# FrancisTheCat/raytracing_c

Measured on AMD Instinct MI355X. Metric: Mray/s, higher is better.
Workload: dtype f32; 1 GPU; helmet.glb 1920x1080, 256 spp, 8 bounces (BASELINE.json configs[2]); partition=single GPU

## Files before the change

### include/rt_hip.h

```cpp
#ifndef RT_HIP_H
#define RT_HIP_H

#include "rt_raytracer.h"
#include "rt_materials.h"

#ifdef __cplusplus
extern "C" {
#endif

extern char const *rt_last_error(void);
extern void        rt_clear_error(void);

extern int rt_init(int device);

extern int rt_set_devices(i32 n_devices, i32 rehearse);
extern i32 rt_device_count(void);


extern void rt_set_seed(u32 seed);
extern u32  rt_get_seed(void);


typedef struct RT_Device_Scene RT_Device_Scene;

// ... 207 lines not shown

extern i64 rt_guided_upsample_work_bytes(i32 width, i32 height);
extern int rt_guided_upsample(i32 width, i32 height, RT_Upsample_Params const *params, void const *d_color_low,
                              void const *d_coverage_low, void const *d_albedo_low, void const *d_normal_low,
                              void const *d_position_low, void const *d_coverage, void const *d_albedo, void const *d_normal,
                              void const *d_position, void *d_out, void *d_image, void *d_work, void *stream);
extern int rt_guided_upsample_host(i32 width, i32 height, RT_Upsample_Params const *params, f32 const *color_low,
                                   RT_Features const *low, RT_Features const *full, f32 *out, u8 *image);
extern int rt_render_upsampled(Scene const *scene, Image const *image, isize samples, isize max_bounces,
                               RT_Upsample_Params const *upsample_params, RT_Guided_Params const *guided_params, f32 *linear_low,
                               f32 *linear_upsampled, f32 *linear_out);


extern int rt_render_accumulate_chunks(RT_Device_Scene *dscene, RT_Render_Params const *params, i32 n_list, i32 const *chunks,
                                       void *d_accum, void *stream);
extern int rt_adaptive_merge(i32 width, i32 height, i32 n, i32 n_list, i32 const *chunks, void *d_accum, void *d_fresh, void *d_err,
                             void *stream);
extern int rt_resolve_adaptive(i32 width, i32 height, void const *d_chunk_samples, void const *d_accum, void *d_image, void *d_linear,
                               void *d_sample_map, void *stream);

typedef struct {
  i32 min_samples;
  i32 max_samples;
  f32 threshold;
  i32 reserved;
} RT_Adaptive_Params;

extern int rt_render_adaptive(Scene const *scene, Image const *image, RT_Adaptive_Params const *ap, isize max_bounces, f32 *linear,
                              u64 *accum, i32 *chunk_samples);

extern int rt_get_counters(RT_Counters *out);
extern int rt_get_skipped_root_visits(u64 *out);
extern int rt_get_leafless_paths(u64 *out);
extern int rt_get_fused_root_visits(u64 *out);
extern int rt_get_shade_taps_form(void);
extern int rt_materials_share_taps(f32 const *mats, i32 n_materials);

typedef struct {
  f32 stamp_ms, upload_ms, enqueue_ms, gpu_prep_ms, gpu_path_ms, gpu_resolve_ms, gpu_copy_ms, total_ms;
  f32 verify_ms;
  f32 gather_ms;
  i32 n_devices;
  i32 slowest_device;
} RT_Frame_Timing;
extern int rt_get_frame_timing(RT_Frame_Timing *out);

extern f32 rt_last_kernel_ms(void);

extern void rt_kernel_timing_reset(void);
extern f32  rt_kernel_timing_mean_ms(i32 *n_launches);

extern int rt_math_contract(void);


#ifdef __cplusplus
}
#endif

#endif
```

### raytracing_c_amd/csrc/rt_dev.hip.h

```cpp
#ifndef RT_DEV_HIP_H
#define RT_DEV_HIP_H

#include <hip/hip_runtime.h>
#include <stdint.h>

#include "rt_device.h"
#include "../../include/rt_math.h"

#define RT_BLOCK_WAVES 4
#define RT_BLOCK_THREADS (RT_BLOCK_WAVES * 64)

struct Ray3 {
  rt_v3 o, d;
  float inv_x, inv_y, inv_z;
  bool  fast;
};

__device__ __forceinline__ rt_v3 slab_bias3(const Ray3 &r) {
#ifdef RT_MATH_NO_FMA
  return rt_v3_make(0.0f, 0.0f, 0.0f);
#else
  float px, py, pz;
  asm volatile("v_mul_f32 %0, %1, %2" : "=v"(px) : "v"(r.o.x), "v"(r.inv_x));
  asm volatile("v_mul_f32 %0, %1, %2" : "=v"(py) : "v"(r.o.y), "v"(r.inv_y));
// ... 1201 lines not shown
  surv &= surv - 1u;
  const int k2 = (int)__builtin_ctz(surv);
  const int e2 = as_i(slab_entry_ordered(r, bs, nbase, k2, nx, ny, nz, hit_t));
  const uint32_t f2 = 1u - (((uint32_t)e2 + 0x00800000u) >> 31);
  int e3 = 0x7F800000, k3 = 0;
  uint32_t f3 = 0;
  LGM_FEW("four_begin");
  if (n == 4) {
    surv &= surv - 1u;
    k3 = (int)__builtin_ctz(surv);
      e3 = as_i(slab_entry_ordered(r, bs, nbase, k3, nx, ny, nz, hit_t));
    f3 = 1u - (((uint32_t)e3 + 0x00800000u) >> 31);
  }
  LGM_FEW("four_end");
  const int e[4] = {e0, e1, e2, e3};
  const int kk[4] = {k0, k1, k2, k3};
  int rank[4] = {0, 1, 2, 3};
#pragma unroll
  for (int j = 0; j < 4; j++) {
#pragma unroll
    for (int k = j + 1; k < 4; k++) {
      int kb = (int)((uint32_t)(e[k] - e[j]) >> 31);
      rank[j] += kb;
      rank[k] -= kb;
    }
  }
  uint32_t w = 0;
#pragma unroll
  for (int j = 0; j < 4; j++) w |= (uint32_t)kk[j] << (3 * rank[j]);
  return w | ((f0 + f1 + f2 + f3) << 24);
}
#undef LGM_FEW

__device__ __forceinline__ uint32_t pyramid_cull_tris(const float *leaves, const float *pyr, int g) {
  const int lane = lane_now();
  const float *tb = leaves + (size_t)g * 72 + (lane & 7);
  const float *pl = pyr + RT_PYR_PLANE + ((lane >> 3) & 3) * 4;
  const float ox = pyr[RT_PYR_ORIGIN], oy = pyr[RT_PYR_ORIGIN + 1], oz = pyr[RT_PYR_ORIGIN + 2];
  const float nx = pl[0], ny = pl[1], nz = pl[2];
  const float ax = tb[0], e1x = tb[8], e2x = tb[16], ay = tb[24], e1y = tb[32], e2y = tb[40], az = tb[48], e1z = tb[56], e2z = tb[64];
  const float band = 2.5f * RT_EPS * (fabsf(nx * e1x + ny * e1y + nz * e1z) + fabsf(nx * e2x + ny * e2y + nz * e2z));
  bool outside = true;
#pragma unroll
  for (int v = 0; v < 3; v++) {
    const float vx = v == 0 ? ax : (v == 1 ? ax + e1x : ax + e2x);
    const float vy = v == 0 ? ay : (v == 1 ? ay + e1y : ay + e2y);
    const float vz = v == 0 ? az : (v == 1 ? az + e1z : az + e2z);
    const float px = nx * (vx - ox), py = ny * (vy - oy), pz = nz * (vz - oz);
    const float val = px + py + pz;
    const float extent = fabsf(px) + fabsf(py) + fabsf(pz);
    const float coarse = fabsf(nx) * (fabsf(ox) + fabsf(vx)) + fabsf(ny) * (fabsf(oy) + fabsf(vy)) + fabsf(nz) * (fabsf(oz) + fabsf(vz));
    outside = outside && (val - band > 1e-3f * extent + 1e-6f * coarse);
  }
  const uint32_t m = (uint32_t)__ballot(outside);
  return (m | (m >> 8) | (m >> 16) | (m >> 24)) & 0xFFu;
}

template <bool SHORT_DIV>
__device__ __forceinline__ void tri_test_uniform(const Ray3 &r, rt_v3 a, rt_v3 edge1, rt_v3 edge2, int k, float &best, float &bu, float &bv, int &bi) {
  rt_v3 rxe2 = rt_v3_cross(r.d, edge2);
  float det = rt_v3_dot(edge1, rxe2);
  float inv_det = SHORT_DIV ? rcp_leaf(det) : 1.0f / det;
  rt_v3 s = rt_v3_sub(r.o, a);
  rt_v3 sxe1 = rt_v3_cross(s, edge1);
  float u = inv_det * rt_v3_dot(s, rxe2);
  float v = inv_det * rt_v3_dot(r.d, sxe1);
  float t = inv_det * rt_v3_dot(edge2, sxe1);
  bool miss = (u < -RT_EPS) || (u > 1.0f + RT_EPS) || (v < -RT_EPS) || (u + v > 1.0f + RT_EPS) || (t < RT_EPS);
  if (SHORT_DIV) {
    if (!miss && t < best) { best = t; bi = k; bu = u; bv = v; }
  } else {
    float dist = miss ? RT_INF : t;
    dist = (dist > 0.0f) ? dist : RT_INF;
    if (dist < best) { best = dist; bi = k; bu = u; bv = v; }
  }
}
template <bool SHORT_DIV>
__device__ __forceinline__ bool leaf_test_uniform(const RT_KParams &P, const Ray3 &r, int g, uint32_t surv, HitRec &hit) {
  float best = RT_INF, bu = 0.0f, bv = 0.0f;
  int   bi = 0;
  cfloat *lb = as_scalar_ptr(P.leaves) + (size_t)g * 72;
  while (surv) {
    const int k0 = (int)__builtin_ctz(surv);
    surv &= surv - 1u;
    cfloat *t0 = lb + k0;
    tri_test_uniform<SHORT_DIV>(r, rt_v3_make(t0[0], t0[24], t0[48]), rt_v3_make(t0[8], t0[32], t0[56]), rt_v3_make(t0[16], t0[40], t0[64]),
                                k0, best, bu, bv, bi);
// ... 336 lines not shown
```

### raytracing_c_amd/csrc/rt_device.h

```cpp
#ifndef RT_DEVICE_H
#define RT_DEVICE_H

#include <stdint.h>

#define RT_NODE_F4   12
#define RT_LEAF_F4   18
#define RT_TRI_F4     7
#define RT_MAT_F4     9
#define RT_MAT_FLOATS 36
#define RT_MAX_DEPTH  8

#define RT_LDS_BYTES            (160 * 1024)
#define RT_LDS_NODE_BYTES       208
#define RT_LDS_TABLE_BYTES      64
#define RT_LDS_PERM_LEVEL_BYTES 256
#define RT_LDS_ACC_TILE_BYTES   1536

#define RT_MAT_DISNEY 0
#define RT_MAT_DEBUG  1

#define RT_TILE      8
#define RT_TILE_PIX  64

#define RT_PARK_RECORD_DWORDS (18 * 128)
enum {
  RT_CNT_PATHS = 0, RT_CNT_RAYS, RT_CNT_NODES, RT_CNT_LEAVES, RT_CNT_SHADES, RT_CNT_BG, RT_CNT_TEXTURED,
  RT_CNT_SKIPPED_ROOT,
  RT_CNT_LEDGER,
  RT_CNT_LEAFLESS = 136,
  RT_CNT_FUSED_ROOT,
  RT_N_COUNTERS
};
#define RT_CNT_LEDGER_SLOTS (RT_CNT_LEAFLESS - RT_CNT_LEDGER)



typedef struct {
  uint32_t offset;
  int32_t  width, height, stride;
} RT_DTexture;
#define RT_TEX_TILE_INDEX(x, y, tpr) ((((y) >> 2) * (tpr) + ((x) >> 2)) * 16 + (((y) & 3) << 2) + ((x) & 3))

typedef struct RT_KView {
  float    cam[3][4];
  float    focal_length;
  uint32_t seed;
  uint32_t pad[2];
} RT_KView;

typedef struct {
  const float    *nodes;
  const float    *leaves;
  const float    *tris;
  const float    *mats;
  const RT_DTexture *textures;
  const uint32_t *texels;
  int32_t depth;
  int32_t last_row_offset;
  int32_t bg_texture;
  int32_t n_nodes;
  float cam[3][4];
  float focal_length;
  float inv_width, inv_height, aspect;
// ... 101 lines not shown
```

### raytracing_c_amd/csrc/rt_kernels.hip

```cpp

#include "rt_dev.hip.h"


#ifdef RT_LEDGER
#define RT_LEDGER_WAVES 8192
__device__ uint32_t g_ledger[RT_LEDGER_WAVES * RT_LEDGER_ROW];
__global__ void rt_ledger_reduce_kernel(unsigned long long *counters) {
  const int slot = threadIdx.x;
  if (slot >= LG_N || slot >= RT_LEDGER_ROW) return;
  unsigned long long sum = 0ull;
  for (int w = 0; w < RT_LEDGER_WAVES; w++) sum += g_ledger[w * RT_LEDGER_ROW + slot];
  counters[RT_CNT_LEDGER + slot] = sum;
}
#endif

template <int WAVES, bool LDSN, int MIN_WAVES_PER_SIMD, bool SHORT_DIV, bool VIEWS, bool SHARED_TAPS>
__global__ __launch_bounds__(WAVES * 64, MIN_WAVES_PER_SIMD) void rt_path_kernel_stream(RT_KParams P) {
  extern __shared__ float4 smem[];
  const int lane = threadIdx.x & 63;
  const int wave = threadIdx.x >> 6;
  const int n_lds = LDSN ? P.n_lds_nodes : 0;
  const float4 *lds_nodes = smem;
  const WaveLds L = wave_lds(smem, n_lds, P.depth, wave);
  unsigned long long *acc = L.acc;
// ... 43 lines not shown
  const int leaf_level = P.depth - 1;
  const int thresh = P.sched_thresh;
  const int drain_thresh = P.drain_thresh;
  const int pyr_nodes = LDSN ? P.pyr_nodes : 0;
  const int wave_id = (int)blockIdx.x * WAVES + wave;

  bool queue_open = true;
  int  steal_tries = 0;

  for (;;) {
    LGT0();
    LGM("tile_begin");
    int tile_idx = queue_open ? take_queue_tile(lane, queue_open) : -1;
    if (tile_idx < 0) {
      if (steal_tries >= RT_STEAL_TRIES) break;
      steal_tries += 1;
      LG(LG_JOIN_X, 1);
      tile_idx = join_open_tile(lane, wave_id, steal_tries, n_chunks_tile LG_ARG);
      if (tile_idx < 0) break;
    }

    int tile_x0, tile_y0;
    RT_KViewP vrec = nullptr;
    if (!tile_origin<VIEWS>(lane, tile_idx, n_chunks_tile, tile_x0, tile_y0, vrec)) continue;
    bool tile_root_miss = false;
    if (leaf_level >= 0) {
      typename CamSrc<VIEWS>::type S;
      if constexpr (VIEWS) S = vrec; else S = cold_args();
      tile_root_miss = tile_pyramid(S, P.nodes, smem, pyr_off, lane, tile_x0, tile_y0);
    }
    int n_list = 0;
    int ll_levels = leaf_level, ll_nodes = pyr_nodes, ll_leaf0 = P.last_row_offset;
    asm volatile("" : "+s"(ll_levels), "+s"(ll_nodes), "+s"(ll_leaf0));
    if (ll_levels >= 1 && ll_nodes > 0 && !tile_root_miss) n_list = leafless_walk(smem, lds_nodes, pyr_off, ll_levels, ll_nodes, ll_leaf0);
    const uint32_t rays_before = w_rays;
    LG(LG_TILE_X, 1);
    LGM("tile_end");
    LGT1(LG_CYC_TILE);

    int   pix = 0, bounce = 0;
    uint32_t rng = 0;
    Ray3  ray;
    ray_setup(ray, rt_v3_make(0, 0, 0), rt_v3_make(0, 0, 1));
    rt_v3 tint = rt_v3_make(1, 1, 1), emis = rt_v3_make(0, 0, 0);
    TravState T = RT_TRAV_IDLE;

    bool tile_open = true;
    TileUnits U;
    tile_units_init(U, queue_open);
    int  n_parked = 0;
    uint32_t *park = cold_args()->park;

    if ((tile_root_miss || n_list > 0) && cold_args()->max_bounces > 0) {
      RT_KArgs A = cold_args();
      typename CamSrc<VIEWS>::type S;
      if constexpr (VIEWS) S = vrec; else S = A;
      const int width = A->width, height = A->height, sample_first = A->sample_first, sample_end = A->sample_end;
      const uint32_t n_sb = (uint32_t)A->n_sample_blocks, gmax = (uint32_t)A->grab_max;
      PrimaryParams PP;
      primary_params(PP, S, A);
      ShadeParamsLds SP;
      shade_params(SP, A, false);
      uint32_t *tile_next = A->tile_next, *open_groups = A->open_groups;
      uint32_t n_sky = 0;
      const uint32_t *list = leafless_list(smem, pyr_off, ll_levels);
      const uint32_t list_entry = (n_list > 1 && lane_now() < n_list) ? list[RT_LL_ENTRY + (lane_now() & (RT_LL_MAX - 1))] : 0u;
      for (;;) {
        if (U.c_next >= U.c_end) {
          if (U.u_cur + 1u < U.u_end) {
            U.u_cur += 1u;
          } else {
            uint32_t u0 = 0;
            if (lane == 0) u0 = atomicAdd(&tile_next[tile_idx], U.grab);
            u0 = (uint32_t)__builtin_amdgcn_readfirstlane((int)u0);
            if (u0 >= n_chunks_tile) { tile_open = false; break; }
            U.u_cur = u0;
            U.u_end = u0 + U.grab < n_chunks_tile ? u0 + U.grab : n_chunks_tile;
            if (U.u_end == n_chunks_tile && lane == 0) atomicSub(&open_groups[tile_idx >> 6], 1u);
            if (t_wave_start) t_last_grab = __builtin_amdgcn_s_memrealtime();
            LG(LG_GRAB_X, 1);
            const uint32_t left = n_chunks_tile - U.u_end;
            U.grab = left >= 8u * gmax ? gmax : (left >= 8u && gmax >= 2u ? 2u : 1u);
            U.took_any = true;
          }
          unit_decode(U, tile_x0, tile_y0, shift, unit_paths, n_sb, sample_first, width, height);
          continue;
        }
#ifndef RT_SKY_PATHS
#define RT_SKY_PATHS 1
#endif
        LGM("sky_begin");
        LGT0();
        const int avail = U.c_end - U.c_next;
        const int take = avail < 64 * RT_SKY_PATHS ? avail : 64 * RT_SKY_PATHS;
        const int l = lane_now();
        bool valid[RT_SKY_PATHS];
        int  pxs[RT_SKY_PATHS];
        rt_v3 dirs[RT_SKY_PATHS];
        Ray3 rs[RT_SKY_PATHS];
        bool slow = false;
#pragma unroll
        for (int q = 0; q < RT_SKY_PATHS; q++) {
          const int kq = l + 64 * q;
          const int k = U.c_next + kq;
          pxs[q] = k >> shift;
          const int sm = U.c_s0 + (k & ((1 << shift) - 1));
          const int x = U.c_x0 + pxs[q];
          valid[q] = kq < take && x < width && sm < sample_end;
          rt_v3 o = rt_v3_make(0, 0, 0);
          dirs[q] = rt_v3_make(0, 0, 1);
          if (valid[q]) primary_ray(PP, x, U.c_y, sm, o, dirs[q]);
          ray_setup<SHORT_DIV>(rs[q], o, dirs[q]);
          slow = slow || (valid[q] && !rs[q].fast);
        }
        if (__ballot(slow) != 0ull) break;
        uint32_t nv = 0;
        uint32_t e = (uint32_t)__builtin_amdgcn_readlane((int)list_entry, 1);
        if ((int)e < 0) {
#pragma unroll
          for (int q = 0; q < RT_SKY_PATHS; q++) {
            const Ray3 &r = rs[q];
            const int nx = (as_i(r.inv_x) >> 31) & 96, ny = (as_i(r.inv_y) >> 31) & 96, nz = (as_i(r.inv_z) >> 31) & 96;
            const rt_v3 bs = slab_bias3(r);
            uint32_t entered = valid[q] ? 1u : 0u;
            int i = 1;
            if (q > 0) e = (uint32_t)__builtin_amdgcn_readlane((int)list_entry, 1);
            do {
              const char *cb = reinterpret_cast<const char *>(lds_nodes) + (e & 0xFFFFFu);
              const float t = slab_entry_ordered(r, bs, cb, 0, nx, ny, nz, RT_INF);
              const uint32_t in = ((entered >> ((e >> 20) & 7u)) & 1u) & (t < RT_INF ? 1u : 0u);
              entered |= in << i;
              w_nodes += (uint32_t)__popcll(__ballot(in != 0u));
              i += 1;
              e = (uint32_t)__builtin_amdgcn_readlane((int)list_entry, i);
            } while ((int)e < 0);
          }
        }
#pragma unroll
        for (int q = 0; q < RT_SKY_PATHS; q++) {
          unsigned long long qr = 0ull, qg = 0ull, qb = 0ull;
          if (valid[q]) {
            const rt_v3 bg = background_lookup(SP, dirs[q]);
            const rt_v3 radiance = rt_v3_mul_add(bg, rt_v3_make(1, 1, 1), rt_v3_make(0, 0, 0));
            qr = accum_quantize_dev(radiance.x); qg = accum_quantize_dev(radiance.y); qb = accum_quantize_dev(radiance.z);
          }
          tile_add_samples_grouped(smem, acc_off, U.c_pix0 + pxs[q], U.c_end >= 2 * RT_SKY_ADD_GROUP, valid[q], qr, qg, qb);
          nv += (uint32_t)__popcll(__ballot(valid[q]));
        }
        w_paths += nv; w_rays += nv; w_nodes += nv; w_bgs += nv;
        n_sky += nv;
        LG(LG_SKY_X, 1); LG(LG_SKY_L, nv);
        U.c_next += take;
        LGT1(LG_CYC_SKY);
        LGM("sky_end");
      }
      if (n_sky != 0u && lane == 0) atomicAdd(cold_args()->counters + (tile_root_miss ? RT_CNT_SKIPPED_ROOT : RT_CNT_LEAFLESS), (unsigned long long)n_sky);
    }

    for (;;) {
      {
        LGT0();
        LGM("s_begin");
        LG(LG_S_ITER, 1);
        LaneCounters cn;
        cn.rays = cn.nodes = cn.leaves = cn.shades = cn.bgs = cn.textured = cn.paths = 0;
        bool  done = false, start = false, fresh = false;
        rt_v3 radiance = rt_v3_make(0, 0, 0);
        rt_v3 org = ray.o, dir = ray.d;
        RT_KArgs A = cold_args();
        typename PathShadeParams<SHARED_TAPS>::type SP;
        shade_params(SP, A, true);
#ifdef RT_LEDGER
        { const int n_env = (int)__popcll(__ballot(T.phase == PH_MISS)); LG(LG_ENV_X, n_env != 0); LG(LG_ENV_L, n_env); }
#endif
        LGM("env_begin");
        if (T.phase == PH_MISS) {
          cn.bgs = 1;
          rt_v3 bg = background_lookup(SP, dir);
          radiance = rt_v3_mul_add(bg, tint, emis);
          done = true;
        }
        LGM("env_end");
        bool shade_now = true;
        if (park) {
          const unsigned long long mHit = __ballot(T.phase == PH_HIT);
          const unsigned long long mIdle = __ballot(T.phase == PH_NEED) | __ballot(T.phase == PH_MISS);
          const int h = (int)__popcll(mHit), f = (int)__popcll(mIdle);
          const int back = n_parked < f ? n_parked : f;
          uint32_t *pk = park + (size_t)__builtin_amdgcn_readfirstlane(wave_id) * (RT_PARK_FIELDS * RT_PARK_CAP);
// ... 669 lines not shown
```

### raytracing_c_amd/csrc/rt_launch.cpp

```cpp

#include "rt_host.h"

static std::atomic<int> g_taps_form{-1};

int check_params(RT_Render_Params const *p) {
  if (!p) return rt_fail("render params are NULL");
  if (p->width <= 0 || p->height <= 0) return rt_fail("image size %dx%d is invalid", p->width, p->height);
  if ((int64_t)p->width * p->height > (int64_t)1 << 28) return rt_fail("image %dx%d is too large", p->width, p->height);
  if (p->samples <= 0) return rt_fail("samples must be positive (got %d)", p->samples);
  if (p->max_bounces < 0) return rt_fail("max_bounces must be >= 0 (got %d)", p->max_bounces);
  if (p->world <= 0 || p->rank < 0 || p->rank >= p->world) return rt_fail("rank %d / world %d is invalid", p->rank, p->world);
  if (p->sample_first < 0 || p->sample_count < 0 || p->sample_first + p->sample_count > p->samples)
    return rt_fail("sample range [%d, +%d) outside [0, %d)", p->sample_first, p->sample_count, p->samples);
  return 0;
}

int check_image_size(const char *who, i32 width, i32 height) {
  if (width <= 0 || height <= 0) return rt_fail("%s: image size %dx%d is invalid", who, width, height);
  if ((int64_t)width * height > RT_MAX_PIXELS) return rt_fail("%s: image %dx%d is too large (more than 2^28 pixels)", who, width, height);
  return 0;
}

int check_views(i32 n_views, RT_View const *views, i32 width, i32 height, const char *who) {
  if (n_views <= 0) return rt_fail("%s: n_views must be positive (got %d)", who, n_views);
// ... 418 lines not shown

int copy_image_out(Image const *image, const uint8_t *d_image, int width, int height, hipStream_t stream) {
  size_t pixels = (size_t)width * height;
  if (!image->pixels.data) return 0;
  if (image->components == 3 && image->stride == image->width) {
    HIP_TRY(hipMemcpyAsync(image->pixels.data, d_image, pixels * 3, hipMemcpyDeviceToHost, stream));
    HIP_TRY(hipStreamSynchronize(stream));
  } else {
    std::vector<uint8_t> tmp(pixels * 3);
    HIP_TRY(hipMemcpy(tmp.data(), d_image, pixels * 3, hipMemcpyDeviceToHost));
    for (isize y = 0; y < image->height; y++)
      for (isize x = 0; x < image->width; x++)
        for (int c = 0; c < 3; c++)
          image->pixels.data[image->components * (x + y * image->stride) + c] = tmp[((size_t)y * width + x) * 3 + c];
  }
  return 0;
}

static int get_counter(const char *who, int index, u64 *out) {
  if (!out) return rt_fail("%s: NULL", who);
  Device &D = dev0();
  std::lock_guard<std::mutex> lock(D.mutex);
  if (ensure_device(D) != 0) return -1;
  unsigned long long c[RT_N_COUNTERS];
  if (read_counters(D, c) != 0) return -1;
  *out = c[index];
  return 0;
}

extern "C" int rt_get_skipped_root_visits(u64 *out) { return get_counter("rt_get_skipped_root_visits", RT_CNT_SKIPPED_ROOT, out); }

extern "C" int rt_get_leafless_paths(u64 *out) { return get_counter("rt_get_leafless_paths", RT_CNT_LEAFLESS, out); }

extern "C" int rt_get_fused_root_visits(u64 *out) { return get_counter("rt_get_fused_root_visits", RT_CNT_FUSED_ROOT, out); }

extern "C" int rt_get_shade_taps_form(void) { return g_taps_form.load(); }

int read_counters(Device &D, unsigned long long c[RT_N_COUNTERS]) {
  HIP_TRY(hipDeviceSynchronize());
  if (!D.last_counters) { memset(c, 0, RT_N_COUNTERS * sizeof(unsigned long long)); return 0; }
  HIP_TRY(hipMemcpy(c, D.last_counters, RT_N_COUNTERS * sizeof(unsigned long long), hipMemcpyDeviceToHost));
  return 0;
}

extern "C" int rt_get_counters(RT_Counters *out) {
  if (!out) return rt_fail("rt_get_counters: NULL");
  {
    std::lock_guard<std::mutex> lk(g_multi_mutex);
    if (g_multi_counters_valid) { *out = g_multi_counters; return 0; }
  }
  Device &D = dev0();
  std::lock_guard<std::mutex> lock(D.mutex);
  if (ensure_device(D) != 0) return -1;
  unsigned long long c[RT_N_COUNTERS];
  if (read_counters(D, c) != 0) return -1;
  out->paths = c[RT_CNT_PATHS];
  out->rays = c[RT_CNT_RAYS];
  out->node_visits = c[RT_CNT_NODES];
  out->leaf_visits = c[RT_CNT_LEAVES];
  out->shades = c[RT_CNT_SHADES];
  out->backgrounds = c[RT_CNT_BG];
  out->textured = c[RT_CNT_TEXTURED];
  return 0;
}

static float timed_slot_ms(Workspace &W, size_t slot) {
// ... 34 lines not shown
```

### raytracing_c_amd/csrc/rt_tile.hip.h

```cpp
#ifndef RT_TILE_HIP_H
#define RT_TILE_HIP_H

typedef const RT_KView __attribute__((address_space(4))) *RT_KViewP;
template <bool VIEWS> struct CamSrc { typedef RT_KArgs type; };
template <> struct CamSrc<true> { typedef RT_KViewP type; };

__device__ __forceinline__ int take_queue_tile(const int lane, bool &queue_open) {
  RT_KArgs A = cold_args();
  uint32_t pos = 0;
  if (lane == 0) pos = atomicAdd(A->work_head, 1u);
  pos = (uint32_t)__builtin_amdgcn_readfirstlane((int)pos);
  const uint32_t *order = A->order;
  if (pos < (uint32_t)A->n_tiles) return order ? (int)order[pos] : (int)pos;
  queue_open = false;
  return -1;
}

__device__ __forceinline__ int join_open_tile(const int lane, const int wave_id, const int steal_tries, const uint32_t n_chunks_tile,
                                              uint32_t *lg = nullptr) {
  LGT0();
  int tile_idx = -1;
  RT_KArgs A = cold_args();
  const int n_tiles = A->n_tiles;
  const uint32_t *open_groups = A->open_groups, *tile_next = A->tile_next;
// ... 91 lines not shown
  for (int q = 0; q < 4; q++) {
    rt_v3 n = rt_v3_cross(c[q], c[(q + 1) & 3]);
    if (rt_v3_dot(n, c[(q + 2) & 3]) > 0.0f) n = rt_v3_scale(n, -1.0f);
    pn[q] = n;
  }
  float *pyr = lds_at(smem, pyr_off);
  if (lane == 0) {
#pragma unroll
    for (int q = 0; q < 4; q++) { pyr[RT_PYR_PLANE + q * 4 + 0] = pn[q].x; pyr[RT_PYR_PLANE + q * 4 + 1] = pn[q].y; pyr[RT_PYR_PLANE + q * 4 + 2] = pn[q].z; }
    pyr[RT_PYR_ORIGIN] = o.x; pyr[RT_PYR_ORIGIN + 1] = o.y; pyr[RT_PYR_ORIGIN + 2] = o.z;
  }
  if (lane < RT_PYR_CACHE_WORDS) reinterpret_cast<uint32_t *>(pyr)[RT_PYR_LEAF_CACHE + lane] = 0u;
  bool may_hit = false;
  if (lane < 8) {
    const float *nb = nodes + lane;
    rt_v3 lo = rt_v3_make(nb[0] - o.x, nb[8] - o.y, nb[16] - o.z);
    rt_v3 hi = rt_v3_make(nb[24] - o.x, nb[32] - o.y, nb[40] - o.z);
    bool outside = child_box_empty(nb);
#pragma unroll
    for (int q = 0; q < 4; q++) {
      rt_v3 n = pn[q];
      float lox = n.x * lo.x, hix = n.x * hi.x, loy = n.y * lo.y, hiy = n.y * hi.y, loz = n.z * lo.z, hiz = n.z * hi.z;
      float nearest = fminf(lox, hix) + fminf(loy, hiy) + fminf(loz, hiz);
      float extent = fmaxf(fabsf(lox), fabsf(hix)) + fmaxf(fabsf(loy), fabsf(hiy)) + fmaxf(fabsf(loz), fabsf(hiz));
      float coarse = fabsf(n.x) * (fabsf(o.x) + fmaxf(fabsf(nb[0]), fabsf(nb[24]))) + fabsf(n.y) * (fabsf(o.y) + fmaxf(fabsf(nb[8]), fabsf(nb[32]))) +
                     fabsf(n.z) * (fabsf(o.z) + fmaxf(fabsf(nb[16]), fabsf(nb[40])));
      if (nearest > 1e-3f * extent + 1e-6f * coarse) outside = true;
    }
    may_hit = !outside;
  }
  return __ballot(may_hit) == 0ull;
}

#define RT_LL_MAX   8
#define RT_LL_ENTRY 0
#define RT_LL_NODE  RT_LL_MAX
__device__ __forceinline__ uint32_t *leafless_list(float4 *smem, const int pyr_off, const int levels) {
  return reinterpret_cast<uint32_t *>(lds_at(smem, pyr_off) - levels * (RT_LDS_PERM_LEVEL_BYTES / 4));
}
__device__ __forceinline__ int leafless_walk(float4 *smem, const float4 *lds_nodes, const int pyr_off, const int levels, const int n_nodes,
                                             const int leaf0) {
  const float *pyr = lds_at(smem, pyr_off);
  uint32_t *list = leafless_list(smem, pyr_off, levels);
  int n_list = 1;
  for (int head = 0; head < n_list; head++) {
    const int nd = head ? __builtin_amdgcn_readfirstlane((int)list[RT_LL_NODE + head]) : 0;
    const uint32_t surv = 0xFFu & ~pyramid_cull_mask(lds_nodes, pyr, nd);
    if (lane_now() == 0) reinterpret_cast<uint32_t *>(lds_at(smem, pyr_off))[RT_PYR_NODE_CACHE + (nd & 31)] = ((uint32_t)(nd + 1) << 8) | (0xFFu & ~surv);
    if (surv) {
      const int ns = (int)__popc(surv);
      if (8 * nd + 1 >= leaf0 || 8 * nd + 8 >= n_nodes || ns > 4 || n_list + ns > RT_LL_MAX) return 0;
      const int k = lane_now();
      if (k < 8 && ((surv >> k) & 1u)) {
        const int at = n_list + (int)__popc(surv & ((1u << k) - 1u));
        list[RT_LL_ENTRY + at] = (uint32_t)(nd * RT_LDS_NODE_BYTES + k * 4) | ((uint32_t)head << 20) | 0x80000000u;
        list[RT_LL_NODE + at] = (uint32_t)(8 * nd + 1 + k);
      }
      n_list += ns;
    }
  }
  return n_list;
}

struct TileUnits {
  uint32_t u_cur, u_end, grab;
  int  c_next, c_end;
  int  c_x0, c_y, c_pix0, c_s0;
  bool took_any;
};
__device__ __forceinline__ void tile_units_init(TileUnits &U, const bool queue_open) {
  U.c_next = U.c_end = U.c_x0 = U.c_y = U.c_pix0 = U.c_s0 = 0;
  U.u_cur = U.u_end = 0;
  U.grab = queue_open ? (uint32_t)cold_args()->grab_max : 1u;
  U.took_any = false;
}

__device__ __forceinline__ bool grab_units(const int lane, const int tile_idx, const uint32_t n_chunks_tile, uint32_t *tile_next,
                                           uint32_t *open_groups, const uint32_t gmax, TileUnits &U, const unsigned long long t_wave_start,
                                           unsigned long long &t_last_grab, uint32_t *lg = nullptr) {
  uint32_t u0 = 0;
  if (lane == 0) u0 = atomicAdd(&tile_next[tile_idx], U.grab);
  u0 = (uint32_t)__builtin_amdgcn_readfirstlane((int)u0);
  if (u0 >= n_chunks_tile) return false;
  U.u_cur = u0;
  U.u_end = u0 + U.grab < n_chunks_tile ? u0 + U.grab : n_chunks_tile;
  if (U.u_end == n_chunks_tile && lane == 0) atomicSub(&open_groups[tile_idx >> 6], 1u);
  if (t_wave_start) t_last_grab = __builtin_amdgcn_s_memrealtime();
  LG(LG_GRAB_X, 1);
// ... 86 lines not shown
```

### raytracing_c_amd/ctypes_abi.py

```python
import ctypes as C

import numpy as np

isize = C.c_ssize_t
f32 = C.c_float


class Vec2(C.Structure):
    _fields_ = [("x", f32), ("y", f32)]


class Vec3(C.Structure):
    _fields_ = [("x", f32), ("y", f32), ("z", f32)]


class Matrix_4x4(C.Structure):
    _fields_ = [("rows", (f32 * 4) * 4)]


class Byte_Slice(C.Structure):
    _fields_ = [("data", C.c_void_p), ("len", isize)]


class Image(C.Structure):
# ... 186 lines not shown
assert C.sizeof(Triangle) == 112
assert C.sizeof(Triangle_AOS) == 112
assert C.sizeof(Hit) == 88
assert C.sizeof(PBR_Shader_Data) == 80

TRIANGLE_DTYPE = np.dtype([("positions", "<f4", (3, 3)), ("normals", "<f4", (3, 3)), ("tex_coords", "<f4", (3, 2)),
                           ("shader_data", "<u8"), ("shader_proc", "<u8")])
assert TRIANGLE_DTYPE.itemsize == 112

EXPORTED_SYMBOLS = [
    "render_thread_proc", "rendering_context_is_finished", "rendering_context_finish", "lightmap_bake", "render",
    "denoise_image",
    "scene_init", "scene_init_sah", "scene_init_gpu", "rt_scene_alloc", "rt_scene_free", "scene_load_bytes", "scene_save_bytes", "scene_file_size",
    "rt_scene_slot_map", "scene_refit", "scene_refit_gpu",
    "disney_shader_proc", "debug_shader_proc", "sample_background",
    "rt_last_error", "rt_clear_error", "rt_init", "rt_set_seed", "rt_get_seed",
    "rt_set_devices", "rt_device_count", "rt_math_contract",
    "rt_scene_verify", "rt_scene_touch", "rt_scene_set_static", "rt_get_frame_timing",
    "rt_scene_upload", "rt_scene_release", "rt_scene_invalidate", "rt_scene_device_bytes", "rt_set_camera",
    "rt_device_scene_keep_geometry", "rt_scene_keep_geometry", "rt_scene_has_kept_geometry",
    "rt_chunk_count", "rt_chunk_owner", "rt_local_chunk_count", "rt_max_local_chunk_count", "rt_local_chunk_list", "rt_render_accumulate", "rt_resolve", "rt_untile",
    "rt_denoise", "rt_render_frame", "rt_frame_begin", "rt_frame_end", "rt_render_views", "rt_render_accumulate_views",
    "rt_query_closest", "rt_query_occluded", "rt_scene_hits", "rt_scene_closest", "rt_scene_occluded", "rt_get_query_counters",
    "rt_render_accumulate_features", "rt_resolve_features", "rt_render_features",
    "rt_render_accumulate_features_motion", "rt_resolve_motion", "rt_render_features_motion",
    "rt_guided_work_bytes", "rt_guided_denoise", "rt_guided_denoise_host", "rt_render_denoised",
    "rt_temporal_history_bytes", "rt_temporal_accumulate", "rt_temporal_accumulate_host", "rt_history_create", "rt_history_reset",
    "rt_history_destroy", "rt_history_set_motion", "rt_render_temporal",
    "rt_temporal_moments_bytes", "rt_temporal_accumulate_moments", "rt_temporal_accumulate_moments_host",
    "rt_temporal_accumulate_motion", "rt_temporal_accumulate_motion_host",
    "rt_guided_variance_work_bytes", "rt_guided_denoise_variance", "rt_guided_denoise_variance_host", "rt_render_svgf",
    "rt_guided_upsample_work_bytes", "rt_guided_upsample", "rt_guided_upsample_host", "rt_render_upsampled",
    "rt_render_accumulate_chunks", "rt_adaptive_merge", "rt_resolve_adaptive", "rt_render_adaptive",
    "rt_get_counters", "rt_get_skipped_root_visits", "rt_get_leafless_paths", "rt_get_fused_root_visits", "rt_get_shade_taps_form", "rt_materials_share_taps", "rt_last_kernel_ms", "rt_kernel_timing_reset", "rt_kernel_timing_mean_ms",
]

DIAG_ONLY_SYMBOLS = [
    "rt_diag_set_tokens", "rt_diag_multi_fault", "rt_set_pipeline", "rt_get_pipeline", "rt_set_wavefront_capacity", "rt_get_wave_times", "rt_get_ledger",
    "rt_diag_device_bytes_live", "rt_diag_release_staging", "rt_diag_cached_scene",
    "rt_test_math", "rt_test_rcp_sweep", "rt_test_srgb_sweep", "rt_test_env_sweep", "rt_test_quantize_sweep", "rt_test_encode_sweep", "rt_test_group_sum", "rt_test_sky_add_group", "rt_test_node_order", "rt_test_trace", "rt_test_trace_stream",
    "rt_test_tile_order", "rt_test_texture", "rt_test_shade", "rt_test_shade_hit", "rt_test_feature_hit", "rt_test_brdf", "rt_test_background", "rt_test_primary_ray",
]
```

### raytracing_c_amd/native.py

```python
import ctypes as C
import os

from . import ctypes_abi as abi

_HERE = os.path.dirname(os.path.abspath(__file__))
LIB_PATH = os.environ.get("RT_LIB_PATH") or os.path.join(_HERE, "librt_hip.so")
DIAG_PATH = os.path.join(_HERE, "librt_hip_diag.so")


class NativeLibraryMissing(RuntimeError):
    pass


def _preload_hip_runtime():
    import importlib.util
    import sys
    if os.environ.get("RT_HIP_RUNTIME", "torch") != "torch":
        return
    if "torch" in sys.modules:
        return
    try:
        spec = importlib.util.find_spec("torch")
    except (ImportError, ValueError):
        spec = None
# ... 135 lines not shown
        d.rt_render_svgf.argtypes = [P(abi.Scene), P(abi.Image), abi.isize, abi.isize, vp, P(abi.RT_Temporal_Params),
                                     P(abi.RT_Variance_Params), P(abi.RT_Guided_Params), vp, vp, vp, vp]
    if hasattr(d, "rt_render_upsampled"):
        d.rt_guided_upsample_work_bytes.argtypes = [C.c_int32, C.c_int32]
        d.rt_guided_upsample_work_bytes.restype = C.c_int64
        d.rt_guided_upsample.argtypes = [C.c_int32, C.c_int32, P(abi.RT_Upsample_Params)] + [vp] * 13
        d.rt_guided_upsample_host.argtypes = [C.c_int32, C.c_int32, P(abi.RT_Upsample_Params), vp, P(abi.RT_Features),
                                              P(abi.RT_Features), vp, vp]
        d.rt_render_upsampled.argtypes = [P(abi.Scene), P(abi.Image), abi.isize, abi.isize, P(abi.RT_Upsample_Params),
                                          P(abi.RT_Guided_Params), vp, vp, vp]
    if hasattr(d, "rt_render_adaptive"):
        d.rt_render_accumulate_chunks.argtypes = [vp, P(abi.RT_Render_Params), C.c_int32, vp, vp, vp]
        d.rt_adaptive_merge.argtypes = [C.c_int32] * 4 + [vp] * 5
        d.rt_resolve_adaptive.argtypes = [C.c_int32, C.c_int32] + [vp] * 6
        d.rt_render_adaptive.argtypes = [P(abi.Scene), P(abi.Image), P(abi.RT_Adaptive_Params), abi.isize, vp, vp, vp]
    if hasattr(d, "rt_scene_keep_geometry"):
        d.rt_device_scene_keep_geometry.argtypes = [vp, vp]
        d.rt_scene_keep_geometry.argtypes = [P(abi.Scene)]
        d.rt_scene_has_kept_geometry.argtypes = [P(abi.Scene)]
        d.rt_render_accumulate_features_motion.argtypes = [vp, P(abi.RT_Render_Params), vp, vp, vp]
        d.rt_resolve_motion.argtypes = [P(abi.RT_Render_Params), vp, vp, vp]
        d.rt_render_features_motion.argtypes = [P(abi.Scene), C.c_int32, C.c_int32, abi.isize, abi.isize, P(abi.RT_Features), vp, vp, vp]
        d.rt_temporal_accumulate_motion.argtypes = ([C.c_int32, C.c_int32, P(abi.RT_Temporal_Params), P(abi.Camera), P(abi.Camera)]
                                                    + [vp] * 10 + [P(abi.RT_Variance_Params)] + [vp] * 5)
        d.rt_temporal_accumulate_motion_host.argtypes = [C.c_int32, C.c_int32, P(abi.RT_Temporal_Params), P(abi.Camera), P(abi.Camera),
                                                         vp, P(abi.RT_Features), P(abi.RT_History_Planes), P(abi.RT_History_Planes),
                                                         vp, vp, vp, P(abi.RT_Variance_Params), vp, vp, vp, vp]
        d.rt_history_set_motion.argtypes = [vp, C.c_int]
    d.rt_get_counters.argtypes = [P(abi.RT_Counters)]
    if hasattr(d, "rt_get_skipped_root_visits"):
        d.rt_get_skipped_root_visits.argtypes = [P(C.c_uint64)]
    if hasattr(d, "rt_get_leafless_paths"):
        d.rt_get_leafless_paths.argtypes = [P(C.c_uint64)]
    if hasattr(d, "rt_get_fused_root_visits"):
        d.rt_get_fused_root_visits.argtypes = [P(C.c_uint64)]
    if hasattr(d, "rt_get_shade_taps_form"):
        d.rt_get_shade_taps_form.argtypes = []
        d.rt_materials_share_taps.argtypes = [vp, C.c_int32]
    d.rt_math_contract.restype = C.c_int
    d.rt_last_kernel_ms.restype = C.c_float
    d.rt_kernel_timing_reset.restype = None
    d.rt_kernel_timing_mean_ms.argtypes = [P(C.c_int32)]
    d.rt_kernel_timing_mean_ms.restype = C.c_float
    d.rt_set_devices.argtypes = [C.c_int32, C.c_int32]
    d.rt_device_count.restype = C.c_int32
    d.rt_scene_verify.argtypes = [P(abi.Scene)]
    d.rt_scene_touch.argtypes = [P(abi.Scene), vp, C.c_size_t]
    d.rt_scene_set_static.argtypes = [P(abi.Scene), C.c_int32]
    d.rt_scene_set_static.restype = None
    d.rt_get_frame_timing.argtypes = [P(abi.RT_Frame_Timing)]
    d.render_thread_proc.argtypes = [P(abi.Rendering_Context)]
    d.render_thread_proc.restype = None
    d.rendering_context_is_finished.argtypes = [P(abi.Rendering_Context)]
    d.rendering_context_is_finished.restype = C.c_bool
    d.rendering_context_finish.argtypes = [P(abi.Rendering_Context)]
    d.rendering_context_finish.restype = None
    d.render.argtypes = [P(abi.Scene), P(abi.Image), abi.isize, abi.isize]
    d.lightmap_bake.argtypes = [P(abi.Image), P(abi.Scene), abi.isize]
    d.lightmap_bake.restype = None
    d.denoise_image.argtypes = [P(abi.Image), P(abi.Image), abi.isize]
    d.denoise_image.restype = None
    d.rt_denoise.argtypes = [C.c_int32, C.c_int32, vp, vp, vp]


def _declare_diag(d):
    vp = C.c_void_p
# ... 47 lines not shown
```

### raytracing_c_amd/tile_classes.py

```python
import numpy as np

F = np.float32


def lds_nodes(n_nodes, depth, wg_waves=16):
    per_wave = max(depth, 1) * 256 + 1536
    room = (160 * 1024 - 64 - wg_waves * per_wave) // 208
    return min(n_nodes, max(room, 0))


def tile_pyramids(cam_rows, focal_length, width, height):
    cam = np.asarray(cam_rows, F).reshape(-1, 4)[:3]
    ty, tx = (height + 7) // 8, (width + 7) // 8
    inv_w, inv_h, asp = F(1.0) / F(width), F(1.0) / F(height), F(width) / F(height)
    m = F(0.05)
    x0 = (np.arange(tx, dtype=F) * F(8))[None, :]
    y0 = (np.arange(ty, dtype=F) * F(8))[:, None]
    ux0 = (x0 - F(0.5) - m) * F(2.0) * inv_w - F(1.0)
    ux1 = (x0 + F(7.5) + m) * F(2.0) * inv_w - F(1.0)
    uy0 = (y0 - F(0.5) - m) * F(2.0) * inv_h - F(1.0)
    uy1 = (y0 + F(7.5) + m) * F(2.0) * inv_h - F(1.0)
    c = np.zeros((ty, tx, 4, 3), F)
    for q in range(4):
        cx = np.broadcast_to((ux1 if q in (1, 2) else ux0) * asp, (ty, tx))
        cy = np.broadcast_to(-(uy1 if q >= 2 else uy0), (ty, tx))
        cz = F(-focal_length)
        for i in range(3):
            c[:, :, q, i] = cam[i, 0] * cx + cam[i, 1] * cy + cam[i, 2] * cz
    pn = np.zeros((ty, tx, 4, 3), F)
    for q in range(4):
        n = np.cross(c[:, :, q], c[:, :, (q + 1) & 3]).astype(F)
        flip = np.sum(n * c[:, :, (q + 2) & 3], axis=-1) > 0
        n[flip] = -n[flip]
        pn[:, :, q] = n
    return pn, cam[:, 3].copy()


def cull_masks(nodes, node_idx, pn, origin, margin=1e-3):
    nb = nodes[node_idx]
    mn, mx = nb[:, 0:3, :], nb[:, 3:6, :]
    o = origin.astype(F)[None, :, None]
    empty = np.all(nb == 0, axis=1)
    nrm = pn[:, :, :, None]
    lo = nrm * (mn - o)[:, None]
    hi = nrm * (mx - o)[:, None]
    nearest = np.minimum(lo, hi).sum(axis=2, dtype=F)
    extent = np.maximum(np.abs(lo), np.abs(hi)).sum(axis=2, dtype=F)
    coarse = (np.abs(nrm) * (np.abs(o)[:, None] + np.maximum(np.abs(mn), np.abs(mx))[:, None])).sum(axis=2, dtype=F)
    with np.errstate(invalid="ignore"):
        outside = nearest > F(margin) * extent + F(1e-6) * coarse
    return empty | outside.any(axis=1)


def _cull_chunked(nodes, node, pn, origin, margin, chunk=1 << 17):
    out = np.empty((len(node), 8), bool)
    for a in range(0, len(node), chunk):
        out[a:a + chunk] = cull_masks(nodes, node[a:a + chunk], pn[a:a + chunk], origin, margin)
    return out


def classify_tiles(nodes, depth, cam_rows, focal_length, width, height, margin=1e-3, give_up=64):
    nodes = np.asarray(nodes, F).reshape(-1, 6, 8)
    pn, origin = tile_pyramids(cam_rows, focal_length, width, height)
    ty, tx = pn.shape[:2]
    n_tiles = ty * tx
    pn = pn.reshape(n_tiles, 4, 3)
    leaf_level = depth - 1
    reached_leaf = np.zeros(n_tiles, bool)
    n_listed = np.zeros(n_tiles, np.int64)
    max_surv = np.zeros(n_tiles, np.int64)
    max_node = np.zeros(n_tiles, np.int64)
    root_miss = np.zeros(n_tiles, bool)
    if leaf_level < 0 or len(nodes) == 0:
        reached_leaf[:] = True
    else:
        tile = np.arange(n_tiles)
        node = np.zeros(n_tiles, np.int64)
        for level in range(leaf_level + 1):
            if len(tile) == 0:
                break
            surv = ~_cull_chunked(nodes, node, pn[tile], origin, margin)
            ns = surv.sum(axis=1)
            np.add.at(n_listed, tile, 1)
            np.maximum.at(max_surv, tile, ns)
            np.maximum.at(max_node, tile, node)
            if level == 0:
                root_miss = ns == 0
            if level == leaf_level:
                reached_leaf[tile[ns > 0]] = True
                break
            pi, k = np.nonzero(surv)
            tile, node = tile[pi], 8 * node[pi] + 1 + k
            reached_leaf[n_listed + np.bincount(tile, minlength=n_tiles) > give_up] = True
            keep = ~reached_leaf[tile]
            tile, node = tile[keep], node[keep]
    shape = (ty, tx)
    return dict(root_miss=root_miss.reshape(shape), leafless=(~reached_leaf).reshape(shape), n_listed=n_listed.reshape(shape),
                max_surv=max_surv.reshape(shape), max_node=max_node.reshape(shape))


def classify_scene(hs, width, height, margin=1e-3):
    cam = hs.scene.camera
    rows = [[cam.view_matrix.rows[i][j] for j in range(4)] for i in range(4)]
    return classify_tiles(hs.nodes_array(), hs.depth, rows, cam.focal_length, width, height, margin)
```

Baseline: 24100 Mray/s.

## Extend leafless tile walk to leaf groups whose triangles are all pyramid-culled

The per-tile leafless walk could previously only prove a tile empty above the leaf level. It now descends into leaf groups, culls each group's triangles against the tile pyramid and ignores zero padding slots. When every triangle is culled, the tile is treated as triangleless, so its primary rays skip full traversal. The list capacity grows from 8 to 32 entries, and the parent bitmask widens to 5 bits. The cost is more per-tile setup work and a new counter atomic, and culling accuracy decides whether skipped rays were truly misses.

```diff
diff --git a/include/rt_hip.h b/include/rt_hip.h
--- a/include/rt_hip.h
+++ b/include/rt_hip.h
@@ -263,6 +263,7 @@
 extern int rt_get_counters(RT_Counters *out);
 extern int rt_get_skipped_root_visits(u64 *out);
 extern int rt_get_leafless_paths(u64 *out);
+extern int rt_get_triangleless_paths(u64 *out);
 extern int rt_get_fused_root_visits(u64 *out);
 extern int rt_get_shade_taps_form(void);
 extern int rt_materials_share_taps(f32 const *mats, i32 n_materials);
diff --git a/raytracing_c_amd/csrc/rt_dev.hip.h b/raytracing_c_amd/csrc/rt_dev.hip.h
--- a/raytracing_c_amd/csrc/rt_dev.hip.h
+++ b/raytracing_c_amd/csrc/rt_dev.hip.h
@@ -1257,7 +1257,8 @@
 }
 #undef LGM_FEW
 
-__device__ __forceinline__ uint32_t pyramid_cull_tris(const float *leaves, const float *pyr, int g) {
+template <bool PADDING = false>
+__device__ __forceinline__ uint32_t pyramid_cull_tris(const float *leaves, const float *pyr, int g, uint32_t *padding = nullptr) {
   const int lane = lane_now();
   const float *tb = leaves + (size_t)g * 72 + (lane & 7);
   const float *pl = pyr + RT_PYR_PLANE + ((lane >> 3) & 3) * 4;
@@ -1278,6 +1279,10 @@
     outside = outside && (val - band > 1e-3f * extent + 1e-6f * coarse);
   }
   const uint32_t m = (uint32_t)__ballot(outside);
+  if (PADDING) {
+    const bool zero = ax == 0.0f && e1x == 0.0f && e2x == 0.0f && ay == 0.0f && e1y == 0.0f && e2y == 0.0f && az == 0.0f && e1z == 0.0f && e2z == 0.0f;
+    *padding = (uint32_t)__ballot(zero) & 0xFFu;
+  }
   return (m | (m >> 8) | (m >> 16) | (m >> 24)) & 0xFFu;
 }
 
diff --git a/raytracing_c_amd/csrc/rt_device.h b/raytracing_c_amd/csrc/rt_device.h
--- a/raytracing_c_amd/csrc/rt_device.h
+++ b/raytracing_c_amd/csrc/rt_device.h
@@ -29,6 +29,7 @@
   RT_CNT_LEDGER,
   RT_CNT_LEAFLESS = 136,
   RT_CNT_FUSED_ROOT,
+  RT_CNT_TRIANGLELESS,
   RT_N_COUNTERS
 };
 #define RT_CNT_LEDGER_SLOTS (RT_CNT_LEAFLESS - RT_CNT_LEDGER)
diff --git a/raytracing_c_amd/csrc/rt_kernels.hip b/raytracing_c_amd/csrc/rt_kernels.hip
--- a/raytracing_c_amd/csrc/rt_kernels.hip
+++ b/raytracing_c_amd/csrc/rt_kernels.hip
@@ -99,7 +99,7 @@
     int n_list = 0;
     int ll_levels = leaf_level, ll_nodes = pyr_nodes, ll_leaf0 = P.last_row_offset;
     asm volatile("" : "+s"(ll_levels), "+s"(ll_nodes), "+s"(ll_leaf0));
-    if (ll_levels >= 1 && ll_nodes > 0 && !tile_root_miss) n_list = leafless_walk(smem, lds_nodes, pyr_off, ll_levels, ll_nodes, ll_leaf0);
+    if (ll_levels >= 1 && ll_nodes > 0 && !tile_root_miss) n_list = leafless_walk(smem, lds_nodes, pyr_off, ll_levels, ll_nodes, ll_leaf0, cold_args()->leaves);
     const uint32_t rays_before = w_rays;
     LG(LG_TILE_X, 1);
     LGM("tile_end");
@@ -131,7 +131,7 @@
       uint32_t *tile_next = A->tile_next, *open_groups = A->open_groups;
       uint32_t n_sky = 0;
       const uint32_t *list = leafless_list(smem, pyr_off, ll_levels);
-      const uint32_t list_entry = (n_list > 1 && lane_now() < n_list) ? list[RT_LL_ENTRY + (lane_now() & (RT_LL_MAX - 1))] : 0u;
+      const uint32_t list_entry = (n_list > 1 && lane_now() < n_list) ? list[RT_LL_ENTRY + (lane_now() & 31)] : 0u;
       for (;;) {
         if (U.c_next >= U.c_end) {
           if (U.u_cur + 1u < U.u_end) {
@@ -195,9 +195,11 @@
             do {
               const char *cb = reinterpret_cast<const char *>(lds_nodes) + (e & 0xFFFFFu);
               const float t = slab_entry_ordered(r, bs, cb, 0, nx, ny, nz, RT_INF);
-              const uint32_t in = ((entered >> ((e >> 20) & 7u)) & 1u) & (t < RT_INF ? 1u : 0u);
+              const uint32_t in = ((entered >> ((e >> 20) & 31u)) & 1u) & (t < RT_INF ? 1u : 0u);
               entered |= in << i;
-              w_nodes += (uint32_t)__popcll(__ballot(in != 0u));
+              const uint32_t n_in = (uint32_t)__popcll(__ballot(in != 0u));
+              if (e & RT_LL_GROUP) w_leaves += n_in;
+              else w_nodes += n_in;
               i += 1;
               e = (uint32_t)__builtin_amdgcn_readlane((int)list_entry, i);
             } while ((int)e < 0);
@@ -222,6 +224,8 @@
         LGM("sky_end");
       }
       if (n_sky != 0u && lane == 0) atomicAdd(cold_args()->counters + (tile_root_miss ? RT_CNT_SKIPPED_ROOT : RT_CNT_LEAFLESS), (unsigned long long)n_sky);
+      if (n_sky != 0u && (__ballot((list_entry & RT_LL_GROUP) != 0u) & ~1ull) != 0ull && lane == 0)
+        atomicAdd(cold_args()->counters + RT_CNT_TRIANGLELESS, (unsigned long long)n_sky);
     }
 
     for (;;) {
diff --git a/raytracing_c_amd/csrc/rt_launch.cpp b/raytracing_c_amd/csrc/rt_launch.cpp
--- a/raytracing_c_amd/csrc/rt_launch.cpp
+++ b/raytracing_c_amd/csrc/rt_launch.cpp
@@ -474,6 +474,8 @@
 
 extern "C" int rt_get_leafless_paths(u64 *out) { return get_counter("rt_get_leafless_paths", RT_CNT_LEAFLESS, out); }
 
+extern "C" int rt_get_triangleless_paths(u64 *out) { return get_counter("rt_get_triangleless_paths", RT_CNT_TRIANGLELESS, out); }
+
 extern "C" int rt_get_fused_root_visits(u64 *out) { return get_counter("rt_get_fused_root_visits", RT_CNT_FUSED_ROOT, out); }
 
 extern "C" int rt_get_shade_taps_form(void) { return g_taps_form.load(); }
diff --git a/raytracing_c_amd/csrc/rt_tile.hip.h b/raytracing_c_amd/csrc/rt_tile.hip.h
--- a/raytracing_c_amd/csrc/rt_tile.hip.h
+++ b/raytracing_c_amd/csrc/rt_tile.hip.h
@@ -147,28 +147,42 @@
   return __ballot(may_hit) == 0ull;
 }
 
-#define RT_LL_MAX   8
+#define RT_LL_MAX   32
 #define RT_LL_ENTRY 0
 #define RT_LL_NODE  RT_LL_MAX
+#define RT_LL_GROUP 0x40000000u
+static_assert(2 * RT_LL_MAX * 4 <= RT_LDS_PERM_LEVEL_BYTES && RT_LL_MAX <= 32, "the list is one row of the perm stack, `entered` one word");
 __device__ __forceinline__ uint32_t *leafless_list(float4 *smem, const int pyr_off, const int levels) {
   return reinterpret_cast<uint32_t *>(lds_at(smem, pyr_off) - levels * (RT_LDS_PERM_LEVEL_BYTES / 4));
 }
 __device__ __forceinline__ int leafless_walk(float4 *smem, const float4 *lds_nodes, const int pyr_off, const int levels, const int n_nodes,
-                                             const int leaf0) {
+                                             const int leaf0, const float *leaves) {
   const float *pyr = lds_at(smem, pyr_off);
   uint32_t *list = leafless_list(smem, pyr_off, levels);
   int n_list = 1;
   for (int head = 0; head < n_list; head++) {
     const int nd = head ? __builtin_amdgcn_readfirstlane((int)list[RT_LL_NODE + head]) : 0;
+    if (nd >= leaf0) continue;
     const uint32_t surv = 0xFFu & ~pyramid_cull_mask(lds_nodes, pyr, nd);
     if (lane_now() == 0) reinterpret_cast<uint32_t *>(lds_at(smem, pyr_off))[RT_PYR_NODE_CACHE + (nd & 31)] = ((uint32_t)(nd + 1) << 8) | (0xFFu & ~surv);
     if (surv) {
       const int ns = (int)__popc(surv);
-      if (8 * nd + 1 >= leaf0 || 8 * nd + 8 >= n_nodes || ns > 4 || n_list + ns > RT_LL_MAX) return 0;
+      const bool groups = 8 * nd + 1 >= leaf0;
+      if ((!groups && 8 * nd + 8 >= n_nodes) || ns > 4 || n_list + ns > RT_LL_MAX) return 0;
+      if (groups) {
+        for (uint32_t m = surv; m; m &= m - 1u) {
+          const int g = 8 * nd + 1 + (int)__builtin_ctz(m) - leaf0;
+          if ((uint32_t)g >= 0x800000u) return 0;
+          uint32_t padding = 0u;
+          const uint32_t cull = pyramid_cull_tris<true>(leaves, pyr, g, &padding);
+          if (lane_now() == 0) reinterpret_cast<uint32_t *>(lds_at(smem, pyr_off))[RT_PYR_LEAF_CACHE + (g & 7)] = ((0x800000u | (uint32_t)g) << 8) | cull;
+          if ((0xFFu & ~(cull | padding)) != 0u) return 0;
+        }
+      }
       const int k = lane_now();
       if (k < 8 && ((surv >> k) & 1u)) {
         const int at = n_list + (int)__popc(surv & ((1u << k) - 1u));
-        list[RT_LL_ENTRY + at] = (uint32_t)(nd * RT_LDS_NODE_BYTES + k * 4) | ((uint32_t)head << 20) | 0x80000000u;
+        list[RT_LL_ENTRY + at] = (uint32_t)(nd * RT_LDS_NODE_BYTES + k * 4) | ((uint32_t)head << 20) | (groups ? RT_LL_GROUP : 0u) | 0x80000000u;
         list[RT_LL_NODE + at] = (uint32_t)(8 * nd + 1 + k);
       }
       n_list += ns;
diff --git a/raytracing_c_amd/ctypes_abi.py b/raytracing_c_amd/ctypes_abi.py
--- a/raytracing_c_amd/ctypes_abi.py
+++ b/raytracing_c_amd/ctypes_abi.py
@@ -242,7 +242,7 @@
     "rt_guided_variance_work_bytes", "rt_guided_denoise_variance", "rt_guided_denoise_variance_host", "rt_render_svgf",
     "rt_guided_upsample_work_bytes", "rt_guided_upsample", "rt_guided_upsample_host", "rt_render_upsampled",
     "rt_render_accumulate_chunks", "rt_adaptive_merge", "rt_resolve_adaptive", "rt_render_adaptive",
-    "rt_get_counters", "rt_get_skipped_root_visits", "rt_get_leafless_paths", "rt_get_fused_root_visits", "rt_get_shade_taps_form", "rt_materials_share_taps", "rt_last_kernel_ms", "rt_kernel_timing_reset", "rt_kernel_timing_mean_ms",
+    "rt_get_counters", "rt_get_skipped_root_visits", "rt_get_leafless_paths", "rt_get_triangleless_paths", "rt_get_fused_root_visits", "rt_get_shade_taps_form", "rt_materials_share_taps", "rt_last_kernel_ms", "rt_kernel_timing_reset", "rt_kernel_timing_mean_ms",
 ]
 
 DIAG_ONLY_SYMBOLS = [
diff --git a/raytracing_c_amd/native.py b/raytracing_c_amd/native.py
--- a/raytracing_c_amd/native.py
+++ b/raytracing_c_amd/native.py
@@ -191,6 +191,8 @@
         d.rt_get_skipped_root_visits.argtypes = [P(C.c_uint64)]
     if hasattr(d, "rt_get_leafless_paths"):
         d.rt_get_leafless_paths.argtypes = [P(C.c_uint64)]
+    if hasattr(d, "rt_get_triangleless_paths"):
+        d.rt_get_triangleless_paths.argtypes = [P(C.c_uint64)]
     if hasattr(d, "rt_get_fused_root_visits"):
         d.rt_get_fused_root_visits.argtypes = [P(C.c_uint64)]
     if hasattr(d, "rt_get_shade_taps_form"):
diff --git a/raytracing_c_amd/tile_classes.py b/raytracing_c_amd/tile_classes.py
--- a/raytracing_c_amd/tile_classes.py
+++ b/raytracing_c_amd/tile_classes.py
@@ -52,6 +52,32 @@
     return empty | outside.any(axis=1)
 
 
+def cull_tris(soa, group, pn, origin, margin=1e-3, zero_culled=True):
+    soa = np.asarray(soa, F)
+    n_groups = soa.shape[1] // 8
+    inside = np.asarray(group) < n_groups
+    slots = np.where(inside, group, 0)[:, None] * 8 + np.arange(8)[None, :]
+    v = soa[:, slots] * inside[None, :, None].astype(F)
+    a = np.stack([v[0], v[3], v[6]], axis=1)
+    e1 = np.stack([v[1], v[4], v[7]], axis=1) - a
+    e2 = np.stack([v[2], v[5], v[8]], axis=1) - a
+    zero = np.all(v == 0, axis=0)
+    o = origin.astype(F)[None, None, :, None]
+    nrm = pn[:, :, :, None]
+    with np.errstate(invalid="ignore", over="ignore"):
+        band = F(2.5e-4) * (np.abs((nrm * e1[:, None]).sum(axis=2, dtype=F)) + np.abs((nrm * e2[:, None]).sum(axis=2, dtype=F)))
+        outside = np.ones(band.shape, bool)
+        for vert in (a, a + e1, a + e2):
+            vert = vert[:, None]
+            p = nrm * (vert - o)
+            val = p.sum(axis=2, dtype=F)
+            extent = np.abs(p).sum(axis=2, dtype=F)
+            coarse = (np.abs(nrm) * (np.abs(o) + np.abs(vert))).sum(axis=2, dtype=F)
+            outside &= val - band > F(margin) * extent + F(1e-6) * coarse
+    culled = outside.any(axis=1)
+    return culled | zero if zero_culled else culled
+
+
 def _cull_chunked(nodes, node, pn, origin, margin, chunk=1 << 17):
     out = np.empty((len(node), 8), bool)
     for a in range(0, len(node), chunk):
@@ -59,7 +85,7 @@
     return out
 
 
-def classify_tiles(nodes, depth, cam_rows, focal_length, width, height, margin=1e-3, give_up=64):
+def classify_tiles(nodes, depth, cam_rows, focal_length, width, height, margin=1e-3, give_up=64, tris=None, zero_culled=True):
     nodes = np.asarray(nodes, F).reshape(-1, 6, 8)
     pn, origin = tile_pyramids(cam_rows, focal_length, width, height)
     ty, tx = pn.shape[:2]
@@ -71,6 +97,9 @@
     max_surv = np.zeros(n_tiles, np.int64)
     max_node = np.zeros(n_tiles, np.int64)
     root_miss = np.zeros(n_tiles, bool)
+    n_groups = np.zeros(n_tiles, np.int64)
+    has_tri = np.zeros(n_tiles, bool)
+    leaf0 = (8 ** max(depth, 0) - 1) // 7
     if leaf_level < 0 or len(nodes) == 0:
         reached_leaf[:] = True
     else:
@@ -88,6 +117,14 @@
                 root_miss = ns == 0
             if level == leaf_level:
                 reached_leaf[tile[ns > 0]] = True
+                if tris is not None:
+                    pi, k = np.nonzero(surv)
+                    np.add.at(n_groups, tile[pi], 1)
+                    group = 8 * node[pi] + 1 + k - leaf0
+                    for a in range(0, len(pi), 1 << 15):
+                        b = slice(a, a + (1 << 15))
+                        kept = ~cull_tris(tris, group[b], pn[tile[pi[b]]], origin, margin, zero_culled)
+                        has_tri[tile[pi[b]][kept.any(axis=1)]] = True
                 break
             pi, k = np.nonzero(surv)
             tile, node = tile[pi], 8 * node[pi] + 1 + k
@@ -95,11 +132,16 @@
             keep = ~reached_leaf[tile]
             tile, node = tile[keep], node[keep]
     shape = (ty, tx)
-    return dict(root_miss=root_miss.reshape(shape), leafless=(~reached_leaf).reshape(shape), n_listed=n_listed.reshape(shape),
-                max_surv=max_surv.reshape(shape), max_node=max_node.reshape(shape))
+    out = dict(root_miss=root_miss.reshape(shape), leafless=(~reached_leaf).reshape(shape), n_listed=n_listed.reshape(shape),
+               max_surv=max_surv.reshape(shape), max_node=max_node.reshape(shape))
+    if tris is not None:
+        out.update(triangleless=((n_groups > 0) & ~has_tri).reshape(shape), n_groups=n_groups.reshape(shape),
+                   n_entries=(n_listed - 1 + n_groups).reshape(shape))
+    return out
 
 
-def classify_scene(hs, width, height, margin=1e-3):
+def classify_scene(hs, width, height, margin=1e-3, triangles=False, zero_culled=True):
     cam = hs.scene.camera
     rows = [[cam.view_matrix.rows[i][j] for j in range(4)] for i in range(4)]
-    return classify_tiles(hs.nodes_array(), hs.depth, rows, cam.focal_length, width, height, margin)
+    return classify_tiles(hs.nodes_array(), hs.depth, rows, cam.focal_length, width, height, margin,
+                          tris=hs.soa_array() if triangles else None, zero_culled=zero_culled)
```

New measurement: 24540 Mray/s, median of 6. 1.8% higher.
